# rpng/open_vins

Hardware: NVIDIA H100
Metric: msckf_updates_per_sec (higher is better)
Workload: dtype f64

## Files before the change

open_vins_b200/csrc/k_triangulate.cu:

```cuda
#include "geom.cuh"

__global__ void k_cam_poses(const DevFrame *fr, DevCamPoses *cc) {
  OVB_PDL_ENTER();
  int idx = blockIdx.x * blockDim.x + threadIdx.x;
  int total = fr->n_cams * fr->n_clones;
  if (idx >= total)
    return;
  int cam = idx / fr->n_clones, cl = idx % fr->n_clones;
  dm3 R_ItoC = ld_m3(fr->cam_R[cam]);
  dv3 p_IinC = ld_v3(fr->cam_p[cam]);
  dm3 R_GtoI = ld_m3(fr->clone_R[cl]);
  dv3 p_IinG = ld_v3(fr->clone_p[cl]);
  dm3 R = mul33(R_ItoC, R_GtoI);
  dv3 p = sub3(p_IinG, mTv3(R, p_IinC));
#pragma unroll
  for (int i = 0; i < 9; i++)
    cc->cc_R[cam][cl][i] = R.m[i];
  cc->cc_p[cam][cl][0] = p.x;
  cc->cc_p[cam][cl][1] = p.y;
  cc->cc_p[cam][cl][2] = p.z;
}

void launch_cam_poses(ovb_ctx *ctx) {
  int total = OVB_MAX_CAMS * OVB_MAX_CLONES;
  k_cam_poses<<<(total + 127) / 128, 128, 0, ctx->stream>>>(ctx->d_frame, ctx->d_cc);
}

#define TRI_MAX_WARPS 8
#define TRI_PITCH 33
template <int NV> __device__ __forceinline__ void seq_add(double (&s)[NV], const double (&c)[NV], int count, double *wbuf) {
  const int lane = threadIdx.x & 31;
#pragma unroll
  for (int k = 0; k < NV; k++)
    wbuf[k * TRI_PITCH + lane] = c[k];
  __syncwarp();
  double a = 0.0;
#pragma unroll
  for (int k = 0; k < NV; k++)
    a = (lane == k) ? s[k] : a;
  if (lane < NV) {
    const double *row = wbuf + lane * TRI_PITCH;
    for (int l = 0; l < count; l++)
      a += row[l];
  }
#pragma unroll
  for (int k = 0; k < NV; k++)
    s[k] = __shfl_sync(0xffffffffu, a, k);
  __syncwarp();
}

struct Rel {
  dm3 R;
  dv3 t;
  dv3 q;
};
__device__ __forceinline__ Rel rel_pose(const DevCamPoses *fr, int cam, int cl, const dm3 &R_GtoA, dv3 p_AinG) {
  dm3 Rc = ld_m3(fr->cc_R[cam][cl]);
  dv3 pc = ld_v3(fr->cc_p[cam][cl]);
  Rel r;
  r.R = mul33T(Rc, R_GtoA);
  r.t = mv3(R_GtoA, sub3(pc, p_AinG));
  r.q = negmv3(r.R, r.t);
  return r;
}

__device__ __forceinline__ double lm_cost(const DevCamPoses *fr, const BlobView &bv, int m0, int m1, int lane, const dm3 &R_GtoA, dv3 p_AinG,
                                          double alpha, double beta, double rho, double *wbuf) {
  double err[1] = {0.0};
  for (int base = m0; base < m1; base += 32) {
    const int i = base + lane;
    double c[1] = {0.0};
    if (i < m1) {
      Rel r = rel_pose(fr, bv.cam[i], bv.clone[i], R_GtoA, p_AinG);
      double hi1 = r.R.m[0] * alpha + r.R.m[1] * beta + r.R.m[2] + rho * r.q.x;
      double hi2 = r.R.m[3] * alpha + r.R.m[4] * beta + r.R.m[5] + rho * r.q.y;
      double hi3 = r.R.m[6] * alpha + r.R.m[7] * beta + r.R.m[8] + rho * r.q.z;
      float z0 = (float)(hi1 / hi3), z1 = (float)(hi2 / hi3);
      float r0 = __fsub_rn(bv.uvn[2 * i], z0), r1 = __fsub_rn(bv.uvn[2 * i + 1], z1);
      float nrm = __fsqrt_rn(__fadd_rn(__fmul_rn(r0, r0), __fmul_rn(r1, r1)));
      c[0] = (double)nrm * (double)nrm;
    }
    seq_add<1>(err, c, min(32, m1 - base), wbuf);
  }
  return err[0];
}

__global__ void __launch_bounds__(256) k_triangulate(const DevCamPoses *__restrict__ fr, const DevOpts *__restrict__ dop,
                                                     DevFeat *__restrict__ feats, int n_feats, BlobView bv) {
  OVB_PDL_ENTER();
  __shared__ double tri_stage[TRI_MAX_WARPS][9 * TRI_PITCH];
  double *wbuf = tri_stage[threadIdx.x >> 5];
  int warp = (blockIdx.x * blockDim.x + threadIdx.x) >> 5;
  int lane = threadIdx.x & 31;
  if (warp >= n_feats)
    return;
  DevFeat *F = &feats[warp];
  const ovb_opts &op = dop->o;
  int m0 = F->m0, m1 = F->m1;
  const double qnan = __longlong_as_double(0x7ff8000000000000LL);
  int status = OVB_FEAT_OK;
  dv3 pA = mk3(qnan, qnan, qnan), pG = pA;
  int anchor_cam = -1, anchor_clone = -1;
  if (m1 - m0 < 2) {
    status = OVB_FEAT_FEW_MEAS;
  } else {
    int most = 0;
    anchor_cam = 0;
    for (int k = F->key0; k < F->key1; k++) {
      int key = bv.keys[k];
      int cnt = 0;
      for (int i = m0 + lane; i < m1; i += 32)
        cnt += (bv.cam[i] == key) ? 1 : 0;
#pragma unroll
      for (int o = 16; o > 0; o >>= 1)
        cnt += __shfl_xor_sync(0xffffffffu, cnt, o);
      if (cnt > most) {
        anchor_cam = key;
        most = cnt;
      }
    }
    int ameas = -1;
    for (int i = m0 + lane; i < m1; i += 32)
      if (bv.cam[i] == anchor_cam)
        ameas = i;
#pragma unroll
    for (int o = 16; o > 0; o >>= 1)
      ameas = max(ameas, __shfl_xor_sync(0xffffffffu, ameas, o));
    anchor_clone = bv.clone[ameas];
    dm3 R_GtoA = ld_m3(fr->cc_R[anchor_cam][anchor_clone]);
    dv3 p_AinG = ld_v3(fr->cc_p[anchor_cam][anchor_clone]);
    dv3 p_f;
    if (!op.triangulate_1d) {
      double Ab[9] = {0, 0, 0, 0, 0, 0, 0, 0, 0};
      for (int base = m0; base < m1; base += 32) {
        const int i = base + lane;
        double c[9] = {0, 0, 0, 0, 0, 0, 0, 0, 0};
        if (i < m1) {
          Rel r = rel_pose(fr, bv.cam[i], bv.clone[i], R_GtoA, p_AinG);
          dv3 bi = mTv3(r.R, mk3((double)bv.uvn[2 * i], (double)bv.uvn[2 * i + 1], 1.0));
          double nb = norm3(bi);
          bi = mk3(bi.x / nb, bi.y / nb, bi.z / nb);
          dm3 Bp = skew3(bi);
          dm3 Ai = mulT33(Bp, Bp);
          dv3 Aip = mv3(Ai, r.t);
          c[0] = Ai.m[0], c[1] = Ai.m[1], c[2] = Ai.m[2], c[3] = Ai.m[4], c[4] = Ai.m[5], c[5] = Ai.m[8];
          c[6] = Aip.x, c[7] = Aip.y, c[8] = Aip.z;
        }
        seq_add<9>(Ab, c, min(32, m1 - base), wbuf);
      }
      double A[9] = {Ab[0], Ab[1], Ab[2], Ab[1], Ab[3], Ab[4], Ab[2], Ab[4], Ab[5]};
      double b[3] = {Ab[6], Ab[7], Ab[8]};
      p_f = colpiv_solve3(A, mk3(b[0], b[1], b[2]));
      double condA = cond_sym3(A);
      if (fabs(condA) > op.max_cond_number)
        status = OVB_FEAT_TRI_COND;
      else if (p_f.z < op.min_dist || p_f.z > op.max_dist)
        status = OVB_FEAT_TRI_DEPTH;
      else if (isnan(norm3(p_f)))
        status = OVB_FEAT_TRI_NAN;
    } else {
      dv3 ba = mk3((double)bv.uvn[2 * ameas], (double)bv.uvn[2 * ameas + 1], 1.0);
      double nba = norm3(ba);
      ba = mk3(ba.x / nba, ba.y / nba, ba.z / nba);
      double Ab1[2] = {0.0, 0.0};
      for (int base = m0; base < m1; base += 32) {
        const int i = base + lane;
        double c[2] = {0.0, 0.0};
        if (i < m1 && i != ameas) {
          Rel r = rel_pose(fr, bv.cam[i], bv.clone[i], R_GtoA, p_AinG);
          dv3 bi = mTv3(r.R, mk3((double)bv.uvn[2 * i], (double)bv.uvn[2 * i + 1], 1.0));
          double nb = norm3(bi);
          bi = mk3(bi.x / nb, bi.y / nb, bi.z / nb);
          dm3 Bp = skew3(bi);
          dv3 Bb = mv3(Bp, ba);
          c[0] = dot3(Bb, Bb);
          c[1] = dot3(Bb, mv3(Bp, r.t));
        }
        seq_add<2>(Ab1, c, min(32, m1 - base), wbuf);
      }
      const double A1 = Ab1[0], b1 = Ab1[1];
      double depth = b1 / A1;
      p_f = mk3(depth * ba.x, depth * ba.y, depth * ba.z);
      if (p_f.z < op.min_dist || p_f.z > op.max_dist)
        status = OVB_FEAT_TRI_DEPTH;
      else if (isnan(norm3(p_f)))
        status = OVB_FEAT_TRI_NAN;
    }
    if (status == OVB_FEAT_OK) {
      pA = p_f;
      pG = add3(mTv3(R_GtoA, pA), p_AinG);
    }
    if (status == OVB_FEAT_OK && op.refine_features) {
      double rho = 1 / pA.z;
      double alpha = pA.x / pA.z;
      double beta = pA.y / pA.z;
      double lam = op.init_lamda;
      double eps = 10000;
      int runs = 0;
      bool recompute = true;
      double Hs[6] = {0, 0, 0, 0, 0, 0};
      double g[3] = {0, 0, 0};
      double cost_old = lm_cost(fr, bv, m0, m1, lane, R_GtoA, p_AinG, alpha, beta, rho, wbuf);
      while (runs < op.max_runs && lam < op.max_lamda && eps > op.min_dx) {
        if (recompute) {
#pragma unroll
          for (int k = 0; k < 6; k++)
            Hs[k] = 0.0;
          g[0] = g[1] = g[2] = 0.0;
          double Hg[9] = {0, 0, 0, 0, 0, 0, 0, 0, 0};
          for (int base = m0; base < m1; base += 32) {
            const int i = base + lane;
            double c[9] = {0, 0, 0, 0, 0, 0, 0, 0, 0};
            if (i < m1) {
              Rel r = rel_pose(fr, bv.cam[i], bv.clone[i], R_GtoA, p_AinG);
              double hi1 = r.R.m[0] * alpha + r.R.m[1] * beta + r.R.m[2] + rho * r.q.x;
              double hi2 = r.R.m[3] * alpha + r.R.m[4] * beta + r.R.m[5] + rho * r.q.y;
              double hi3 = r.R.m[6] * alpha + r.R.m[7] * beta + r.R.m[8] + rho * r.q.z;
              double h3sq = hi3 * hi3;
              double H0[3], H1[3];
              H0[0] = (r.R.m[0] * hi3 - hi1 * r.R.m[6]) / h3sq;
              H0[1] = (r.R.m[1] * hi3 - hi1 * r.R.m[7]) / h3sq;
              H0[2] = (r.q.x * hi3 - hi1 * r.q.z) / h3sq;
              H1[0] = (r.R.m[3] * hi3 - hi2 * r.R.m[6]) / h3sq;
              H1[1] = (r.R.m[4] * hi3 - hi2 * r.R.m[7]) / h3sq;
              H1[2] = (r.q.y * hi3 - hi2 * r.q.z) / h3sq;
              float z0 = (float)(hi1 / hi3), z1 = (float)(hi2 / hi3);
              double rd0 = (double)__fsub_rn(bv.uvn[2 * i], z0), rd1 = (double)__fsub_rn(bv.uvn[2 * i + 1], z1);
              c[0] = H0[0] * H0[0] + H1[0] * H1[0];
              c[1] = H0[0] * H0[1] + H1[0] * H1[1];
              c[2] = H0[0] * H0[2] + H1[0] * H1[2];
              c[3] = H0[1] * H0[1] + H1[1] * H1[1];
              c[4] = H0[1] * H0[2] + H1[1] * H1[2];
              c[5] = H0[2] * H0[2] + H1[2] * H1[2];
#pragma unroll
              for (int a = 0; a < 3; a++)
                c[6 + a] = H0[a] * rd0 + H1[a] * rd1;
            }
            seq_add<9>(Hg, c, min(32, m1 - base), wbuf);
          }
#pragma unroll
          for (int k = 0; k < 6; k++)
            Hs[k] = Hg[k];
#pragma unroll
          for (int k = 0; k < 3; k++)
            g[k] = Hg[6 + k];
        }
        double Hl[9] = {Hs[0] * (1.0 + lam), Hs[1], Hs[2], Hs[1], Hs[3] * (1.0 + lam), Hs[4], Hs[2], Hs[4], Hs[5] * (1.0 + lam)};
        dv3 dx = colpiv_solve3(Hl, mk3(g[0], g[1], g[2]));
        double cost = lm_cost(fr, bv, m0, m1, lane, R_GtoA, p_AinG, alpha + dx.x, beta + dx.y, rho + dx.z, wbuf);
        if (cost <= cost_old && (cost_old - cost) / cost_old < op.min_dcost) {
          alpha += dx.x;
          beta += dx.y;
          rho += dx.z;
          eps = 0;
          break;
        }
        if (cost <= cost_old) {
          recompute = true;
          cost_old = cost;
          alpha += dx.x;
          beta += dx.y;
          rho += dx.z;
          runs++;
          lam = lam / op.lam_mult;
          eps = norm3(dx);
        } else {
          recompute = false;
          lam = lam * op.lam_mult;
        }
      }
      pA = mk3(alpha / rho, beta / rho, 1 / rho);
      dv3 q1, q2;
      householder_tangent3(pA, q1, q2);
      double base_line_max = 0.0;
      for (int i = m0 + lane; i < m1; i += 32) {
        dv3 pc = ld_v3(fr->cc_p[bv.cam[i]][bv.clone[i]]);
        dv3 t = mv3(R_GtoA, sub3(pc, p_AinG));
        double a0 = dot3(q1, t), a1 = dot3(q2, t);
        double bl = sqrt(a0 * a0 + a1 * a1);
        if (bl > base_line_max)
          base_line_max = bl;
      }
      base_line_max = warp_max(base_line_max);
      if (pA.z < op.min_dist || pA.z > op.max_dist)
        status = OVB_FEAT_GN_DEPTH;
      else if ((norm3(pA) / base_line_max) > op.max_baseline)
        status = OVB_FEAT_GN_BASELINE;
      else if (isnan(norm3(pA)))
        status = OVB_FEAT_GN_NAN;
      else
        pG = add3(mTv3(R_GtoA, pA), p_AinG);
    }
  }
  if (lane == 0) {
    F->status = status;
    F->anchor_cam = anchor_cam;
    F->anchor_clone = anchor_clone;
    F->p_FinA[0] = pA.x;
    F->p_FinA[1] = pA.y;
    F->p_FinA[2] = pA.z;
    F->p_FinG[0] = pG.x;
    F->p_FinG[1] = pG.y;
    F->p_FinG[2] = pG.z;
    F->chi2 = qnan;
  }
}

void launch_triangulate(ovb_ctx *ctx, int n_feats, BlobView bv) {
  if (n_feats <= 0)
    return;
  int warps_per_cta = (n_feats + ctx->sm_count - 1) / ctx->sm_count;
  warps_per_cta = warps_per_cta < 1 ? 1 : (warps_per_cta > 8 ? 8 : warps_per_cta);
  int grid = (n_feats + warps_per_cta - 1) / warps_per_cta;
  ovb_launch(ctx, k_triangulate, dim3(grid), dim3(warps_per_cta * 32), (size_t)(0), ctx->d_cc, ctx->d_opts, ctx->d_feat, n_feats, bv);
}
```

open_vins_b200/csrc/ovb_api.cu:

```cuda
#include "ovb_internal.cuh"
#include <chrono>
#include <algorithm>
#include <cmath>
#include <cstdio>
#include <cstdlib>
#include <cstring>
#include <new>
#include <vector>

static const double g_chi2_table[OVB_CHI2_TABLE_LEN] = {
#include "chi2_table.inc"
};

unsigned char *ovb_feat_order_ptr(ovb_ctx *ctx) { return ctx->d_feat_order; }

static size_t align_up(size_t v, size_t a) { return (v + a - 1) / a * a; }

extern "C" {

static ovb_status ensure_stage(ovb_ctx *ctx, size_t doubles);

int ovb_abi_version(void) { return OVB_ABI_VERSION; }

double ovb_chi2_quantile95(int dof) {
// ... 96 lines not shown
  ctx->off_opts = align_up(sizeof(DevFrame), 256);
  ctx->off_feat = ctx->off_opts + align_up(sizeof(DevOpts), 256);
  ctx->off_blob = ctx->off_feat + align_up(sizeof(DevFeat) * (size_t)ctx->cfg.max_feats, 256);
  ctx->blob_cap = align_up((size_t)ctx->cfg.max_meas * (1 + 2 + 8 + 8) + (size_t)ctx->cfg.max_feats * OVB_MAX_CAMS + 64, 256);
  ctx->arena_bytes = ctx->off_blob + ctx->blob_cap;
  CK(cudaMalloc(&ctx->d_arena, ctx->arena_bytes));
  CK(cudaMallocHost(&ctx->h_arena, ctx->arena_bytes));
  ctx->d_frame = (DevFrame *)ctx->d_arena;
  ctx->d_opts = (DevOpts *)(ctx->d_arena + ctx->off_opts);
  ctx->d_feat = (DevFeat *)(ctx->d_arena + ctx->off_feat);
  ctx->d_blob = ctx->d_arena + ctx->off_blob;
  ctx->h_frame = (DevFrame *)ctx->h_arena;
  ctx->h_opts = (DevOpts *)(ctx->h_arena + ctx->off_opts);
  ctx->h_feat = (DevFeat *)(ctx->h_arena + ctx->off_feat);
  ctx->h_blob = ctx->h_arena + ctx->off_blob;
  CK(cudaMalloc(&ctx->d_cc, sizeof(DevCamPoses)));
  CK(cudaMalloc(&ctx->d_feat_order, (size_t)ctx->cfg.max_feats * (OVB_MAX_VARS + 1)));
  ctx->info_bytes = align_up(sizeof(DevUpdateInfo), 256);
  CK(cudaMalloc(&ctx->d_info, ctx->info_bytes + sizeof(double) * (size_t)ms));
  ctx->d_dx = (double *)((char *)ctx->d_info + ctx->info_bytes);
  CK(cudaMallocHost(&ctx->h_info, ctx->info_bytes + sizeof(double) * (size_t)ms));
  ctx->h_dx = (double *)((char *)ctx->h_info + ctx->info_bytes);
  CK(cudaMalloc(&ctx->d_chi2_table, sizeof(g_chi2_table)));
  CK(cudaMemcpy(ctx->d_chi2_table, g_chi2_table, sizeof(g_chi2_table), cudaMemcpyHostToDevice));
  ctx->max_rows = ctx->cfg.max_rows > 0 ? ctx->cfg.max_rows : 2 * ctx->cfg.max_meas;
  if (ctx->max_rows < 2 * ctx->cfg.max_meas)
    ctx->max_rows = 2 * ctx->cfg.max_meas;
  int ldcap = std::min(OVB_MAX_COLS, ms) + 8;
  ctx->Hs_cap = (size_t)ctx->max_rows * ldcap;
  CK(cudaMalloc(&ctx->d_Hs, sizeof(double) * ctx->Hs_cap));
  ctx->h_stage = nullptr;
// ... 21 lines not shown
#undef CK
  *out = ctx;
  return OVB_OK;
}

void ovb_destroy(ovb_ctx *ctx) {
  if (ctx)
    for (int i = 0; i < 2 * 96; i++)
      if (ctx->prof_ev[i])
        cudaEventDestroy(ctx->prof_ev[i]);
  if (!ctx)
    return;
  cudaSetDevice(ctx->device);
  if (ctx->stream)
    cudaStreamSynchronize(ctx->stream);
  void *dev[] = {ctx->P[0],   ctx->P[1], ctx->d_arena, ctx->d_cc, ctx->d_feat_order, ctx->d_info, ctx->d_chi2_table, ctx->d_Hs, ctx->d_W[0],
                 ctx->d_W[1], ctx->d_R,  ctx->d_R2,    ctx->d_M,  ctx->d_S,          ctx->d_Y,    ctx->d_w,          ctx->d_scratch,
                 ctx->d_long, ctx->d_dump, ctx->P_snap, ctx->d_flush, ctx->d_Gpart, ctx->d_G, ctx->d_cqw, ctx->d_grp, ctx->d_grp_acc, ctx->d_init, ctx->d_imu, ctx->d_pub};
  for (void *p : dev)
    if (p)
      cudaFree(p);
  void *host[] = {ctx->h_arena, ctx->h_info, ctx->h_stage, ctx->h_grp, ctx->h_init, ctx->h_imu};
  for (void *p : host)
    if (p)
      cudaFreeHost(p);
  for (int i = 0; i < 8; i++)
    if (ctx->ev[i])
      cudaEventDestroy(ctx->ev[i]);
  if (ctx->ev_fork)
    cudaEventDestroy(ctx->ev_fork);
  if (ctx->ev_join)
// ... 826 lines not shown
  stats->ms_total = ctx->stage_ms[5];
}

ovb_status ovb_triangulate(ovb_ctx *ctx, const ovb_frame *frame, const ovb_feat_batch *feats, const ovb_opts *opts, ovb_feat_out *out) {
  if (!ctx || !out)
    return OVB_ERR_ARG;
  OVB_CUDA_CHECK(ctx, cudaSetDevice(ctx->device));
  Packed pk;
  int saveN = ctx->N;
  if (ctx->N == 0)
    ctx->N = ctx->cfg.max_state;
  ovb_status st = pack_inputs(ctx, frame, feats, opts, nullptr, &pk, nullptr, false);
  ctx->N = saveN;
  if (st != OVB_OK)
    return st;
  launch_cam_poses(ctx);
  launch_triangulate(ctx, pk.n_feats, pk.bv);
  OVB_CUDA_CHECK(ctx, cudaGetLastError());
  OVB_CUDA_CHECK(ctx, cudaMemcpyAsync(ctx->h_feat, ctx->d_feat, sizeof(DevFeat) * (size_t)pk.n_feats, cudaMemcpyDeviceToHost, ctx->stream));
  OVB_CUDA_CHECK(ctx, cudaStreamSynchronize(ctx->stream));
  unpack_feats(ctx, pk.n_feats, out);
  return OVB_OK;
}

ovb_status ovb_feature_jacobians(ovb_ctx *ctx, const ovb_frame *frame, const ovb_feat_batch *feats, const ovb_opts *opts, ovb_feat_out *out,
                                 int stage, double *Hf_out, double *Hx_out, double *res_out, int32_t *row_off_out, int32_t *ncols_out,
                                 int32_t *col_index_out, int ld_out) {
  if (!ctx || !out || !row_off_out || !ncols_out || !col_index_out)
    return OVB_ERR_ARG;
  if (ctx->N < 1) {
    snprintf(ctx->err, sizeof(ctx->err), "ovb_feature_jacobians: no covariance loaded (ovb_cov_set)");
    return OVB_ERR_ARG;
  }
  OVB_CUDA_CHECK(ctx, cudaSetDevice(ctx->device));
  Packed pk;
  ovb_status st = pack_inputs(ctx, frame, feats, opts, out, &pk);
  if (st != OVB_OK)
    return st;
  const int F = pk.n_feats, n_all = pk.n_all;
  if (ld_out < n_all)
    return OVB_ERR_ARG;
  *ncols_out = n_all;
  for (int s = 0, c = 0; s < ctx->h_frame->n_slots; s++)
    for (int k = 0; k < ctx->h_frame->slot_size[s]; k++)
      col_index_out[c++] = ctx->h_frame->slot_off[s] + k;
  launch_cam_poses(ctx);
  if (stage == 0) {
    int rows = 2 * pk.n_meas;
    size_t need = (size_t)rows * (OVB_MAX_COLS + 4);
    if (!ctx->d_dump || need > ctx->dump_cap) {
      if (ctx->d_dump)
        cudaFree(ctx->d_dump);
      ctx->dump_cap = need;
      OVB_CUDA_CHECK(ctx, cudaMalloc(&ctx->d_dump, sizeof(double) * ctx->dump_cap));
    }
    ctx->dump_rows = rows;
    OVB_CUDA_CHECK(ctx, cudaMemsetAsync(ctx->d_dump, 0, sizeof(double) * need, ctx->stream));
    launch_feature_system(ctx, F, pk.bv, pk.ldH, 1);
    OVB_CUDA_CHECK(ctx, cudaGetLastError());
    std::vector<double> host(need);
    OVB_CUDA_CHECK(ctx, cudaMemcpyAsync(host.data(), ctx->d_dump, sizeof(double) * need, cudaMemcpyDeviceToHost, ctx->stream));
// ... 92 lines not shown
  int64_t *cnt = ctx->init_counters;
  cnt[0] = cnt[1] = cnt[2] = cnt[3] = 0;
  OVB_CUDA_CHECK(ctx, cudaSetDevice(ctx->device));
  Packed pk;
  const int saveN = ctx->N;
  if (ctx->N == 0)
    ctx->N = ctx->cfg.max_state;
  ovb_status st = pack_inputs(ctx, frame, feats, opts, nullptr, &pk, nullptr, false, feat_rep, sigma_pix, chi2_multipler);
  ctx->N = saveN;
  if (st != OVB_OK)
    return st;
  st = feature_scratch_reserve(ctx, F, false, true);
  if (st != OVB_OK)
    return st;
  cnt[2] += (int64_t)ctx->last_h2d_bytes;
  launch_cam_poses(ctx);
  launch_triangulate(ctx, F, pk.bv);
  OVB_CUDA_CHECK(ctx, cudaGetLastError());
  OVB_CUDA_CHECK(ctx, cudaMemcpyAsync(ctx->h_feat, ctx->d_feat, sizeof(DevFeat) * (size_t)F, cudaMemcpyDeviceToHost, ctx->stream));
  OVB_CUDA_CHECK(ctx, cudaStreamSynchronize(ctx->stream));
  cnt[1]++;
  cnt[3] += (int64_t)(sizeof(DevFeat) * (size_t)F);
  unpack_feats(ctx, F, out);
  if (!ctx->d_init) {
    OVB_CUDA_CHECK(ctx, cudaMalloc(&ctx->d_init, sizeof(DevInitSys)));
    OVB_CUDA_CHECK(ctx, cudaMallocHost(&ctx->h_init, sizeof(DevInitSys)));
  }
  std::vector<int> sched_of(F);
  for (int i = 0; i < F; i++)
    sched_of[ctx->h_feat[i].sched] = i;
  const DevFrame *hf = ctx->h_frame;
// ... 31 lines not shown
      seen |= 1ull << hf->clone_slot[d.anchor_clone];
      if (opts->do_calib_camera_pose && hf->cam_ext_slot[d.anchor_cam] >= 0)
        seen |= 1ull << hf->cam_ext_slot[d.anchor_cam];
    }
    int n = 0;
    for (int s = 0; s < hf->n_slots; s++)
      if ((seen >> s) & 1ull)
        n += hf->slot_size[s];
    if (n > ctx->cfg.max_state)
      return OVB_ERR_CAPACITY;
    cnt[0]++;
    if (moved) {
      copy_frame_values(ctx->h_frame, frame);
      OVB_CUDA_CHECK(ctx, cudaMemcpyAsync(ctx->d_frame, ctx->h_frame, sizeof(DevFrame), cudaMemcpyHostToDevice, ctx->stream));
      cnt[2] += (int64_t)sizeof(DevFrame);
      launch_cam_poses(ctx);
    }
    launch_feature_init(ctx, sched_of[f], pk.bv, pk.ldH);
    launch_init_prep(ctx, f, k, n);
    const int *skip = &ctx->d_init->skip;
    if (!launch_cov_init_augment(ctx, k, n, ctx->d_init->HR, ctx->d_init->Hinv, d.sigma_sq, skip)) {
      snprintf(ctx->err, sizeof(ctx->err), "ovb_slam_delayed_init: covariance augmentation kernel could not be launched (N=%d, k=%d)", N0, k);
      return OVB_ERR_CAPACITY;
    }
    const double *Hdev = ctx->d_Hs + (size_t)d.row0 * pk.ldH;
    const int rows = 2 * (d.m1 - d.m0) - 3;
    int rr = rows;
    if (rows > n) {
      rr = compress_system(ctx, OVB_COMPRESS_CHOLQR2, ctx->d_Hs + (size_t)d.row0 * pk.ldH, rows, n, pk.ldH, ctx->d_R, pk.ldH);
      Hdev = ctx->d_R;
    }
// ... 97 lines not shown
    return n;
  if (mode == OVB_COMPRESS_NORMAL_EQUATIONS && launch_compress_gram(ctx, A, m, n, ldA, Rout, ldR) >= 0)
    return n;
  launch_tsqr(ctx, A, m, n, ldA, Rout, ldR);
  return std::min(m, n);
}

static int enqueue_slam_groups(ovb_ctx *ctx, int n_groups, int ldH);
static int enqueue_update(ovb_ctx *ctx, const Packed &pk, int col_order, cudaEvent_t *ev, bool slam = false) {
  const int N = ctx->N, F = pk.n_feats, ldH = pk.ldH, m_total = pk.m_total, n_all = pk.n_all, n_groups = pk.n_groups;
  const BlobView bv = pk.bv;
  ctx->n_launch = 0;
  ctx->n_launch_tsqr_level = 0;
  ctx->prof_n = 0;
  if (!slam) {
    launch_cam_poses(ctx);
    launch_triangulate(ctx, F, bv);
    ctx->n_launch += 2;
  }
  ctx->n_launch += 1;
  if (ev)
    cudaEventRecord(ev[1], ctx->stream);
  launch_feature_system(ctx, F, bv, ldH, slam ? 2 : 0);
  if (ev)
    cudaEventRecord(ev[2], ctx->stream);
  {
    cudaEventRecord(ctx->ev_fork, ctx->stream);
    cudaStreamWaitEvent(ctx->side_stream, ctx->ev_fork, 0);
    cudaStream_t main_stream = ctx->stream;
    ctx->stream = ctx->side_stream;
    if (slam) {
      launch_column_map_slam(ctx, F, n_groups == 1);
    } else {
// ... 380 lines not shown
  cudaEventRecord(ctx->ev[0], ctx->stream);
  Packed pk;
  ovb_opts o2 = *opts;
  o2.col_order = OVB_COLS_CANONICAL;
  ovb_status st = pack_inputs(ctx, frame, feats, &o2, nullptr, &pk);
  if (st != OVB_OK)
    return st;
  cudaEventRecord(ctx->ev[1], ctx->stream);
  *n_cols = pk.n_all;
  *ld = pk.ldH;
  if ((size_t)pk.n_all * pk.ldH > (size_t)R_cap_doubles)
    return OVB_ERR_CAPACITY;
  ctx->last_pk = pk;
  ctx->n_launch = 0;
  ctx->n_launch_tsqr_level = 0;
  launch_cam_poses(ctx);
  launch_triangulate(ctx, pk.n_feats, pk.bv);
  launch_feature_system(ctx, pk.n_feats, pk.bv, pk.ldH, 0);
  launch_column_map(ctx, pk.n_feats, pk.bv);
  ctx->n_launch += 3;
  if (pk.m_total > 0)
    compress_system(ctx, o2.compress, ctx->d_Hs, pk.m_total, pk.n_all, pk.ldH, R_dev, pk.ldH);
  else
    OVB_CUDA_CHECK(ctx, cudaMemsetAsync(R_dev, 0, sizeof(double) * (size_t)pk.n_all * pk.ldH, ctx->stream));
  cudaEventRecord(ctx->ev[4], ctx->stream);
  OVB_CUDA_CHECK(ctx, cudaGetLastError());
  return OVB_OK;
}

ovb_status ovb_msckf_shard_finish(ovb_ctx *ctx, double *stacked_dev, int n_blocks, ovb_feat_out *out, double *dx, ovb_stats *stats) {
  if (!ctx || !stacked_dev || n_blocks < 1 || !dx || ctx->N < 1)
// ... 344 lines not shown
```

open_vins_b200/csrc/ovb_internal.cuh:

```cuda
#pragma once
#include "../../include/ovb200.h"
#include <cuda_runtime.h>
#include <stdint.h>

#define OVB_BIG_MAX_MEAS 128
#define OVB_MAX_COLS 512
#define OVB_NB 16
#define OVB_CR 256
#define OVB_PROP_MAX_N 64
#define OVB_PROP_STEPS_RESERVE 64
#define OVB_NO_NEG_DIAG 0x7fffffff

struct DevFrame {
  int n_clones, n_cams;
  int n_slots;
  int n_all;
  double clone_R[OVB_MAX_CLONES][9];
  double clone_p[OVB_MAX_CLONES][3];
  double clone_R_fej[OVB_MAX_CLONES][9];
  double clone_p_fej[OVB_MAX_CLONES][3];
  double cam_R[OVB_MAX_CAMS][9];
  double cam_p[OVB_MAX_CAMS][3];
  double cam_intr[OVB_MAX_CAMS][8];
  int cam_model[OVB_MAX_CAMS];
// ... 3 lines not shown
  int clone_slot[OVB_MAX_CLONES];
  int cam_ext_slot[OVB_MAX_CAMS];
  int cam_intr_slot[OVB_MAX_CAMS];
  const struct DevGroup *groups;
  int lm_w;
};

struct DevGroup {
  int f0, f1;
  int row0, rows;
  int n_cols;
  int n_ent;
  int ent[OVB_MAX_VARS + OVB_MAX_COLS];
  int col_state[OVB_MAX_COLS];
  short col_frame[OVB_MAX_COLS];
};

struct DevCamPoses {
  double cc_R[OVB_MAX_CAMS][OVB_MAX_CLONES][9];
  double cc_p[OVB_MAX_CAMS][OVB_MAX_CLONES][3];
};

struct DevOpts {
  ovb_opts o;
  double sigma_pix_sq;
  int rep;
};

struct DevFeat {
  int m0, m1;
  int row0;
  int key0, key1;
  int status;
  int anchor_cam, anchor_clone;
  int sched;
// ... 83 lines not shown
  char err[256];
  int N, ldP;
  double *P[2];
  int cur;
  unsigned char *d_arena, *h_arena;
  size_t arena_bytes, off_opts, off_feat, off_blob;
  DevFrame *d_frame;
  DevOpts *d_opts;
  DevFeat *d_feat;
  unsigned char *d_blob;
  DevFrame *h_frame;
  DevOpts *h_opts;
  DevFeat *h_feat;
  unsigned char *h_blob;
  size_t blob_cap;
  DevCamPoses *d_cc;
  unsigned char *d_feat_order;
  DevUpdateInfo *d_info;
  DevUpdateInfo *h_info;
  double *h_dx;
  double *h_stage;
  size_t stage_cap;
  double *d_chi2_table;
  double *d_Hs;
  size_t Hs_cap;
  double *d_W[2];
  size_t W_cap;
  double *d_R;
  double *d_R2;
  double *d_M;
  double *d_S;
  double *d_Y;
  double *d_w;
  double *d_dx;
  double *d_scratch;
  size_t scratch_per_cta;
  int scratch_ctas;
  double *d_long;
  size_t long_cap;
  double *d_dump;
  size_t dump_cap;
  int dump_rows;
  int max_rows;
  int sm_count;
  size_t info_bytes;
  int attr_done[8];
  int tsqr_pdl;
  int tsqr_cluster;
  int gram_cluster;
  int ekf_chol_dmma;
  mutable float stage_ms[6];
  mutable int stage_pending;
  double host_us[4];
  int replay_enabled, last_pk_valid;
  Packed last_pk;
  int last_col_order;
  double *P_snap;
  void *d_flush;
  DevGroup *d_grp, *h_grp;
  int grp_cap;
  double *d_grp_acc;
// ... 12 lines not shown
  size_t imu_cap;
  int prof_on, prof_n;
  cudaEvent_t prof_ev[2 * 96];
  const void *prof_fn[96];
};

#define OVB_CUDA_CHECK(ctx, call)                                                                                     \
  do {                                                                                                                \
    cudaError_t e_ = (call);                                                                                          \
    if (e_ != cudaSuccess) {                                                                                          \
      snprintf((ctx)->err, sizeof((ctx)->err), "%s:%d %s: %s", __FILE__, __LINE__, #call, cudaGetErrorString(e_));    \
      return OVB_ERR_CUDA;                                                                                            \
    }                                                                                                                 \
  } while (0)

void launch_cam_poses(ovb_ctx *ctx);
void launch_triangulate(ovb_ctx *ctx, int n_feats, BlobView bv);
void launch_feature_system(ovb_ctx *ctx, int n_feats, BlobView bv, int ldH, int mode);
ovb_status feature_scratch_reserve(ovb_ctx *ctx, int n_feats, bool slam, bool init = false);
void launch_feature_init(ovb_ctx *ctx, int sched, BlobView bv, int ldH);
void launch_init_prep(ovb_ctx *ctx, int feat, int k, int n);
void launch_column_map(ovb_ctx *ctx, int n_feats, BlobView bv, int rows_drop = 3);
void launch_column_map_slam(ovb_ctx *ctx, int n_feats, bool full_map);
void launch_tsqr(ovb_ctx *ctx, double *A, int m, int n, int ldA, double *Rout, int ldR);
int launch_compress_gram(ovb_ctx *ctx, const double *A, int m, int n, int ldA, double *Rout, int ldR);
int launch_compress_cholqr2(ovb_ctx *ctx, double *A, int m, int n, int ldA, double *Rout, int ldR);
bool launch_chol_ekf_dmma(ovb_ctx *ctx, double *S, int ldS, int r, const double *res, double *w, double *invdiag, double **Lpk_out,
                          unsigned long long *epoch_out);
bool launch_trsm_rows(ovb_ctx *ctx, double *A, int ldA, int m, int nt, const double *Lpk, unsigned long long epoch);
bool launch_chol_solve_wide(ovb_ctx *ctx, double *S, int ldS, int r, double *w, double *invdiag, double *M, int ldM, int N, bool gate_only);
void launch_reorder_R(ovb_ctx *ctx, const double *Rin, int n_all, int ldRin, double *Rout, int ldRout);
// ... 44 lines not shown
```

Measured before the change: 2576.

## Fuse camera-pose kernel into triangulation and cache relative poses in shared memory

Removes the separate k_cam_poses launch and computes camera poses inline inside the triangulation kernel. Each warp now computes per-measurement relative poses once into dynamic shared memory, and reuses them across the linear solve, every Levenberg-Marquardt pass and the baseline check, instead of recomputing them each time. The LM step also merges the cost and Hessian passes so the initial cost comes from the Hessian pass. The price is that the host must scan the features for the largest measurement count to size shared memory, and large features can limit warps per CTA. An optional compile-time probe adds clock64 phase timing.

```diff
diff --git a/open_vins_b200/csrc/k_triangulate.cu b/open_vins_b200/csrc/k_triangulate.cu
--- a/open_vins_b200/csrc/k_triangulate.cu
+++ b/open_vins_b200/csrc/k_triangulate.cu
@@ -1,46 +1,96 @@
 #include "geom.cuh"
-
-__global__ void k_cam_poses(const DevFrame *fr, DevCamPoses *cc) {
-  OVB_PDL_ENTER();
-  int idx = blockIdx.x * blockDim.x + threadIdx.x;
-  int total = fr->n_cams * fr->n_clones;
-  if (idx >= total)
+#ifdef TRI_PROBE
+#include <cstdio>
+#endif
+
+#ifdef TRI_PROBE
+#define TRI_PROBE_FEATS 8192
+#define TRI_PROBE_EV 40
+struct TriProbe {
+  long long t0, t1;
+  long long beg[TRI_PROBE_EV], end[TRI_PROBE_EV];
+  char lbl[TRI_PROBE_EV];
+  int n, M, acc, rej;
+};
+__device__ TriProbe tri_probe[TRI_PROBE_FEATS];
+__device__ unsigned tri_probe_done;
+#define TRI_P_DECL long long tp_b = clock64(); int tp_n = 0, tp_acc = 0, tp_rej = 0; \
+  TriProbe *tp = (warp < TRI_PROBE_FEATS && lane == 0) ? &tri_probe[warp] : nullptr; if (tp) tp->t0 = tp_b
+#define TRI_P_BEGIN() do { tp_b = clock64(); } while (0)
+#define TRI_P_END(c) do { long long e_ = clock64(); if (tp && tp_n < TRI_PROBE_EV) { tp->beg[tp_n] = tp_b; tp->end[tp_n] = e_; tp->lbl[tp_n] = (c); } tp_n++; } while (0)
+#define TRI_P_ACC() (tp_acc++)
+#define TRI_P_REJ() (tp_rej++)
+#define TRI_P_FINISH() tri_probe_finish(tp, warp, lane, n_feats, tp_n, m1 - m0, tp_acc, tp_rej)
+__device__ __noinline__ void tri_probe_finish(TriProbe *tp, int warp, int lane, int n_feats, int n, int M, int acc, int rej) {
+  if (lane != 0)
     return;
-  int cam = idx / fr->n_clones, cl = idx % fr->n_clones;
+  if (tp) {
+    tp->t1 = clock64();
+    tp->n = n < TRI_PROBE_EV ? n : TRI_PROBE_EV;
+    tp->M = M, tp->acc = acc, tp->rej = rej;
+  }
+  __threadfence();
+  if (atomicAdd(&tri_probe_done, 1u) != (unsigned)n_feats - 1)
+    return;
+  __threadfence();
+  const int nf = n_feats < TRI_PROBE_FEATS ? n_feats : TRI_PROBE_FEATS;
+  int w = 0;
+  long long sum = 0;
+  for (int f = 0; f < nf; f++) {
+    const long long t = tri_probe[f].t1 - tri_probe[f].t0;
+    sum += t;
+    if (t > tri_probe[w].t1 - tri_probe[w].t0)
+      w = f;
+  }
+  const TriProbe &p = tri_probe[w];
+  long long ph[8] = {0, 0, 0, 0, 0, 0, 0, 0};
+  int npass = 0;
+  for (int k = 0; k < p.n; k++) {
+    const long long d = p.end[k] - p.beg[k];
+    const char c = p.lbl[k];
+    ph[c == 'a' ? 0 : c == 'l' ? 1 : c == 'c' ? 2 : (c == 'S' || c == 'H') ? 3 : c == 'A' ? 4 : c == 'R' ? 5 : 6] += d;
+    npass += (c == 'S' || c == 'H' || c == 'A' || c == 'R') ? 1 : 0;
+  }
+  long long tracked = 0;
+  for (int k = 0; k < 7; k++)
+    tracked += ph[k];
+  printf("TRI_PROBE n_feats=%d mean_warp=%lld longest warp=%d M=%d a=%d r=%d passes=%d total=%lld | anchor %lld linear %lld cond %lld "
+         "start+Hessian %lld trial-acc %lld trial-rej %lld baseline %lld other %lld\n",
+         n_feats, sum / nf, w, p.M, p.acc, p.rej, npass, p.t1 - p.t0, ph[0], ph[1], ph[2], ph[3], ph[4], ph[5], ph[6], p.t1 - p.t0 - tracked);
+  for (int k = 0; k < p.n; k++)
+    printf("TRI_PROBE   %c %lld\n", p.lbl[k], p.end[k] - p.beg[k]);
+  tri_probe_done = 0;
+}
+#else
+#define TRI_P_DECL do { } while (0)
+#define TRI_P_BEGIN() do { } while (0)
+#define TRI_P_END(c) do { } while (0)
+#define TRI_P_ACC() do { } while (0)
+#define TRI_P_REJ() do { } while (0)
+#define TRI_P_FINISH() do { } while (0)
+#endif
+
+__device__ __forceinline__ void cam_pose(const DevFrame *fr, int cam, int cl, dm3 &R, dv3 &p) {
   dm3 R_ItoC = ld_m3(fr->cam_R[cam]);
   dv3 p_IinC = ld_v3(fr->cam_p[cam]);
   dm3 R_GtoI = ld_m3(fr->clone_R[cl]);
   dv3 p_IinG = ld_v3(fr->clone_p[cl]);
-  dm3 R = mul33(R_ItoC, R_GtoI);
-  dv3 p = sub3(p_IinG, mTv3(R, p_IinC));
-#pragma unroll
-  for (int i = 0; i < 9; i++)
-    cc->cc_R[cam][cl][i] = R.m[i];
-  cc->cc_p[cam][cl][0] = p.x;
-  cc->cc_p[cam][cl][1] = p.y;
-  cc->cc_p[cam][cl][2] = p.z;
-}
-
-void launch_cam_poses(ovb_ctx *ctx) {
-  int total = OVB_MAX_CAMS * OVB_MAX_CLONES;
-  k_cam_poses<<<(total + 127) / 128, 128, 0, ctx->stream>>>(ctx->d_frame, ctx->d_cc);
-}
-
-#define TRI_MAX_WARPS 8
-#define TRI_PITCH 33
-template <int NV> __device__ __forceinline__ void seq_add(double (&s)[NV], const double (&c)[NV], int count, double *wbuf) {
+  R = mul33(R_ItoC, R_GtoI);
+  p = sub3(p_IinG, mTv3(R, p_IinC));
+}
+
+#define TRI_REL 15
+#define TRI_NC 10
+#define TRI_APOSE 12
+#define TRI_SMEM_LIMIT (227 * 1024)
+
+template <int NV> __device__ __forceinline__ void seq_sum(double (&s)[NV], const double *stg, int pitch, int M) {
   const int lane = threadIdx.x & 31;
-#pragma unroll
-  for (int k = 0; k < NV; k++)
-    wbuf[k * TRI_PITCH + lane] = c[k];
   __syncwarp();
   double a = 0.0;
-#pragma unroll
-  for (int k = 0; k < NV; k++)
-    a = (lane == k) ? s[k] : a;
   if (lane < NV) {
-    const double *row = wbuf + lane * TRI_PITCH;
-    for (int l = 0; l < count; l++)
+    const double *row = stg + lane * pitch;
+    for (int l = 0; l < M; l++)
       a += row[l];
   }
 #pragma unroll
@@ -54,54 +104,89 @@
   dv3 t;
   dv3 q;
 };
-__device__ __forceinline__ Rel rel_pose(const DevCamPoses *fr, int cam, int cl, const dm3 &R_GtoA, dv3 p_AinG) {
-  dm3 Rc = ld_m3(fr->cc_R[cam][cl]);
-  dv3 pc = ld_v3(fr->cc_p[cam][cl]);
+__device__ __forceinline__ void rel_pose_store(const DevFrame *fr, int cam, int cl, const dm3 &R_GtoA, dv3 p_AinG, double *rel, int pitch) {
+  dm3 Rc;
+  dv3 pc;
+  cam_pose(fr, cam, cl, Rc, pc);
   Rel r;
   r.R = mul33T(Rc, R_GtoA);
   r.t = mv3(R_GtoA, sub3(pc, p_AinG));
   r.q = negmv3(r.R, r.t);
-  return r;
-}
-
-__device__ __forceinline__ double lm_cost(const DevCamPoses *fr, const BlobView &bv, int m0, int m1, int lane, const dm3 &R_GtoA, dv3 p_AinG,
-                                          double alpha, double beta, double rho, double *wbuf) {
-  double err[1] = {0.0};
-  for (int base = m0; base < m1; base += 32) {
-    const int i = base + lane;
-    double c[1] = {0.0};
-    if (i < m1) {
-      Rel r = rel_pose(fr, bv.cam[i], bv.clone[i], R_GtoA, p_AinG);
-      double hi1 = r.R.m[0] * alpha + r.R.m[1] * beta + r.R.m[2] + rho * r.q.x;
-      double hi2 = r.R.m[3] * alpha + r.R.m[4] * beta + r.R.m[5] + rho * r.q.y;
-      double hi3 = r.R.m[6] * alpha + r.R.m[7] * beta + r.R.m[8] + rho * r.q.z;
-      float z0 = (float)(hi1 / hi3), z1 = (float)(hi2 / hi3);
-      float r0 = __fsub_rn(bv.uvn[2 * i], z0), r1 = __fsub_rn(bv.uvn[2 * i + 1], z1);
-      float nrm = __fsqrt_rn(__fadd_rn(__fmul_rn(r0, r0), __fmul_rn(r1, r1)));
-      c[0] = (double)nrm * (double)nrm;
-    }
-    seq_add<1>(err, c, min(32, m1 - base), wbuf);
-  }
-  return err[0];
-}
-
-__global__ void __launch_bounds__(256) k_triangulate(const DevCamPoses *__restrict__ fr, const DevOpts *__restrict__ dop,
-                                                     DevFeat *__restrict__ feats, int n_feats, BlobView bv) {
+#pragma unroll
+  for (int k = 0; k < 9; k++)
+    rel[k * pitch] = r.R.m[k];
+  rel[9 * pitch] = r.t.x, rel[10 * pitch] = r.t.y, rel[11 * pitch] = r.t.z;
+  rel[12 * pitch] = r.q.x, rel[13 * pitch] = r.q.y, rel[14 * pitch] = r.q.z;
+}
+__device__ __forceinline__ dm3 rel_R(const double *rel, int pitch) {
+  dm3 R;
+#pragma unroll
+  for (int k = 0; k < 9; k++)
+    R.m[k] = rel[k * pitch];
+  return R;
+}
+__device__ __forceinline__ dv3 rel_t(const double *rel, int pitch) { return mk3(rel[9 * pitch], rel[10 * pitch], rel[11 * pitch]); }
+__device__ __forceinline__ dv3 rel_q(const double *rel, int pitch) { return mk3(rel[12 * pitch], rel[13 * pitch], rel[14 * pitch]); }
+
+template <bool HESS>
+__device__ __forceinline__ void lm_pass(double (&s)[HESS ? TRI_NC : 1], const BlobView &bv, int m0, int M, int lane, const double *rel, double *stg,
+                                        int pitch, double alpha, double beta, double rho) {
+  for (int j = lane; j < M; j += 32) {
+    const int i = m0 + j;
+    const dm3 R = rel_R(rel + j, pitch);
+    const dv3 q = rel_q(rel + j, pitch);
+    double hi1 = R.m[0] * alpha + R.m[1] * beta + R.m[2] + rho * q.x;
+    double hi2 = R.m[3] * alpha + R.m[4] * beta + R.m[5] + rho * q.y;
+    double hi3 = R.m[6] * alpha + R.m[7] * beta + R.m[8] + rho * q.z;
+    float z0 = (float)(hi1 / hi3), z1 = (float)(hi2 / hi3);
+    float r0 = __fsub_rn(bv.uvn[2 * i], z0), r1 = __fsub_rn(bv.uvn[2 * i + 1], z1);
+    float nrm = __fsqrt_rn(__fadd_rn(__fmul_rn(r0, r0), __fmul_rn(r1, r1)));
+    stg[j] = (double)nrm * (double)nrm;
+    if (HESS) {
+      double h3sq = hi3 * hi3;
+      double H0[3], H1[3];
+      H0[0] = (R.m[0] * hi3 - hi1 * R.m[6]) / h3sq;
+      H0[1] = (R.m[1] * hi3 - hi1 * R.m[7]) / h3sq;
+      H0[2] = (q.x * hi3 - hi1 * q.z) / h3sq;
+      H1[0] = (R.m[3] * hi3 - hi2 * R.m[6]) / h3sq;
+      H1[1] = (R.m[4] * hi3 - hi2 * R.m[7]) / h3sq;
+      H1[2] = (q.y * hi3 - hi2 * q.z) / h3sq;
+      double rd0 = (double)r0, rd1 = (double)r1;
+      stg[1 * pitch + j] = H0[0] * H0[0] + H1[0] * H1[0];
+      stg[2 * pitch + j] = H0[0] * H0[1] + H1[0] * H1[1];
+      stg[3 * pitch + j] = H0[0] * H0[2] + H1[0] * H1[2];
+      stg[4 * pitch + j] = H0[1] * H0[1] + H1[1] * H1[1];
+      stg[5 * pitch + j] = H0[1] * H0[2] + H1[1] * H1[2];
+      stg[6 * pitch + j] = H0[2] * H0[2] + H1[2] * H1[2];
+#pragma unroll
+      for (int a = 0; a < 3; a++)
+        stg[(7 + a) * pitch + j] = H0[a] * rd0 + H1[a] * rd1;
+    }
+  }
+  seq_sum<HESS ? TRI_NC : 1>(s, stg, pitch, M);
+}
+
+__global__ void __launch_bounds__(256) k_triangulate(const DevFrame *__restrict__ fr, const DevOpts *__restrict__ dop,
+                                                     DevFeat *__restrict__ feats, int n_feats, BlobView bv, int pitch) {
   OVB_PDL_ENTER();
-  __shared__ double tri_stage[TRI_MAX_WARPS][9 * TRI_PITCH];
-  double *wbuf = tri_stage[threadIdx.x >> 5];
+  extern __shared__ double tri_smem[];
+  double *rel = tri_smem + (size_t)(threadIdx.x >> 5) * ((TRI_REL + TRI_NC) * pitch + TRI_APOSE);
+  double *stg = rel + TRI_REL * pitch;
+  double *apose = stg + TRI_NC * pitch;
   int warp = (blockIdx.x * blockDim.x + threadIdx.x) >> 5;
   int lane = threadIdx.x & 31;
   if (warp >= n_feats)
     return;
+  TRI_P_DECL;
   DevFeat *F = &feats[warp];
   const ovb_opts &op = dop->o;
   int m0 = F->m0, m1 = F->m1;
+  const int M = m1 - m0;
   const double qnan = __longlong_as_double(0x7ff8000000000000LL);
   int status = OVB_FEAT_OK;
   dv3 pA = mk3(qnan, qnan, qnan), pG = pA;
   int anchor_cam = -1, anchor_clone = -1;
-  if (m1 - m0 < 2) {
+  if (M < 2) {
     status = OVB_FEAT_FEW_MEAS;
   } else {
     int most = 0;
@@ -127,31 +212,43 @@
     for (int o = 16; o > 0; o >>= 1)
       ameas = max(ameas, __shfl_xor_sync(0xffffffffu, ameas, o));
     anchor_clone = bv.clone[ameas];
-    dm3 R_GtoA = ld_m3(fr->cc_R[anchor_cam][anchor_clone]);
-    dv3 p_AinG = ld_v3(fr->cc_p[anchor_cam][anchor_clone]);
+    dm3 R_GtoA;
+    dv3 p_AinG;
+    cam_pose(fr, anchor_cam, anchor_clone, R_GtoA, p_AinG);
+    if (lane == 0) {
+#pragma unroll
+      for (int k = 0; k < 9; k++)
+        apose[k] = R_GtoA.m[k];
+      apose[9] = p_AinG.x, apose[10] = p_AinG.y, apose[11] = p_AinG.z;
+    }
+    for (int j = lane; j < M; j += 32)
+      rel_pose_store(fr, bv.cam[m0 + j], bv.clone[m0 + j], R_GtoA, p_AinG, rel + j, pitch);
+    TRI_P_END('a');
+    TRI_P_BEGIN();
     dv3 p_f;
     if (!op.triangulate_1d) {
-      double Ab[9] = {0, 0, 0, 0, 0, 0, 0, 0, 0};
-      for (int base = m0; base < m1; base += 32) {
-        const int i = base + lane;
-        double c[9] = {0, 0, 0, 0, 0, 0, 0, 0, 0};
-        if (i < m1) {
-          Rel r = rel_pose(fr, bv.cam[i], bv.clone[i], R_GtoA, p_AinG);
-          dv3 bi = mTv3(r.R, mk3((double)bv.uvn[2 * i], (double)bv.uvn[2 * i + 1], 1.0));
-          double nb = norm3(bi);
-          bi = mk3(bi.x / nb, bi.y / nb, bi.z / nb);
-          dm3 Bp = skew3(bi);
-          dm3 Ai = mulT33(Bp, Bp);
-          dv3 Aip = mv3(Ai, r.t);
-          c[0] = Ai.m[0], c[1] = Ai.m[1], c[2] = Ai.m[2], c[3] = Ai.m[4], c[4] = Ai.m[5], c[5] = Ai.m[8];
-          c[6] = Aip.x, c[7] = Aip.y, c[8] = Aip.z;
-        }
-        seq_add<9>(Ab, c, min(32, m1 - base), wbuf);
+      double Ab[9];
+      for (int j = lane; j < M; j += 32) {
+        const int i = m0 + j;
+        dv3 bi = mTv3(rel_R(rel + j, pitch), mk3((double)bv.uvn[2 * i], (double)bv.uvn[2 * i + 1], 1.0));
+        double nb = norm3(bi);
+        bi = mk3(bi.x / nb, bi.y / nb, bi.z / nb);
+        dm3 Bp = skew3(bi);
+        dm3 Ai = mulT33(Bp, Bp);
+        dv3 Aip = mv3(Ai, rel_t(rel + j, pitch));
+        const double c[9] = {Ai.m[0], Ai.m[1], Ai.m[2], Ai.m[4], Ai.m[5], Ai.m[8], Aip.x, Aip.y, Aip.z};
+#pragma unroll
+        for (int k = 0; k < 9; k++)
+          stg[k * pitch + j] = c[k];
       }
+      seq_sum<9>(Ab, stg, pitch, M);
       double A[9] = {Ab[0], Ab[1], Ab[2], Ab[1], Ab[3], Ab[4], Ab[2], Ab[4], Ab[5]};
       double b[3] = {Ab[6], Ab[7], Ab[8]};
       p_f = colpiv_solve3(A, mk3(b[0], b[1], b[2]));
+      TRI_P_END('l');
+      TRI_P_BEGIN();
       double condA = cond_sym3(A);
+      TRI_P_END('c');
       if (fabs(condA) > op.max_cond_number)
         status = OVB_FEAT_TRI_COND;
       else if (p_f.z < op.min_dist || p_f.z > op.max_dist)
@@ -162,25 +259,27 @@
       dv3 ba = mk3((double)bv.uvn[2 * ameas], (double)bv.uvn[2 * ameas + 1], 1.0);
       double nba = norm3(ba);
       ba = mk3(ba.x / nba, ba.y / nba, ba.z / nba);
-      double Ab1[2] = {0.0, 0.0};
-      for (int base = m0; base < m1; base += 32) {
-        const int i = base + lane;
+      double Ab1[2];
+      for (int j = lane; j < M; j += 32) {
+        const int i = m0 + j;
         double c[2] = {0.0, 0.0};
-        if (i < m1 && i != ameas) {
-          Rel r = rel_pose(fr, bv.cam[i], bv.clone[i], R_GtoA, p_AinG);
-          dv3 bi = mTv3(r.R, mk3((double)bv.uvn[2 * i], (double)bv.uvn[2 * i + 1], 1.0));
+        if (i != ameas) {
+          dv3 bi = mTv3(rel_R(rel + j, pitch), mk3((double)bv.uvn[2 * i], (double)bv.uvn[2 * i + 1], 1.0));
           double nb = norm3(bi);
           bi = mk3(bi.x / nb, bi.y / nb, bi.z / nb);
           dm3 Bp = skew3(bi);
           dv3 Bb = mv3(Bp, ba);
           c[0] = dot3(Bb, Bb);
-          c[1] = dot3(Bb, mv3(Bp, r.t));
+          c[1] = dot3(Bb, mv3(Bp, rel_t(rel + j, pitch)));
         }
-        seq_add<2>(Ab1, c, min(32, m1 - base), wbuf);
+        stg[j] = c[0];
+        stg[pitch + j] = c[1];
       }
+      seq_sum<2>(Ab1, stg, pitch, M);
       const double A1 = Ab1[0], b1 = Ab1[1];
       double depth = b1 / A1;
       p_f = mk3(depth * ba.x, depth * ba.y, depth * ba.z);
+      TRI_P_END('l');
       if (p_f.z < op.min_dist || p_f.z > op.max_dist)
         status = OVB_FEAT_TRI_DEPTH;
       else if (isnan(norm3(p_f)))
@@ -197,58 +296,28 @@
       double lam = op.init_lamda;
       double eps = 10000;
       int runs = 0;
-      bool recompute = true;
-      double Hs[6] = {0, 0, 0, 0, 0, 0};
-      double g[3] = {0, 0, 0};
-      double cost_old = lm_cost(fr, bv, m0, m1, lane, R_GtoA, p_AinG, alpha, beta, rho, wbuf);
+      double s[TRI_NC];
+      TRI_P_BEGIN();
+      lm_pass<true>(s, bv, m0, M, lane, rel, stg, pitch, alpha, beta, rho);
+      TRI_P_END('S');
+      double cost_old = s[0];
+      bool recompute = false;
       while (runs < op.max_runs && lam < op.max_lamda && eps > op.min_dx) {
         if (recompute) {
-#pragma unroll
-          for (int k = 0; k < 6; k++)
-            Hs[k] = 0.0;
-          g[0] = g[1] = g[2] = 0.0;
-          double Hg[9] = {0, 0, 0, 0, 0, 0, 0, 0, 0};
-          for (int base = m0; base < m1; base += 32) {
-            const int i = base + lane;
-            double c[9] = {0, 0, 0, 0, 0, 0, 0, 0, 0};
-            if (i < m1) {
-              Rel r = rel_pose(fr, bv.cam[i], bv.clone[i], R_GtoA, p_AinG);
-              double hi1 = r.R.m[0] * alpha + r.R.m[1] * beta + r.R.m[2] + rho * r.q.x;
-              double hi2 = r.R.m[3] * alpha + r.R.m[4] * beta + r.R.m[5] + rho * r.q.y;
-              double hi3 = r.R.m[6] * alpha + r.R.m[7] * beta + r.R.m[8] + rho * r.q.z;
-              double h3sq = hi3 * hi3;
-              double H0[3], H1[3];
-              H0[0] = (r.R.m[0] * hi3 - hi1 * r.R.m[6]) / h3sq;
-              H0[1] = (r.R.m[1] * hi3 - hi1 * r.R.m[7]) / h3sq;
-              H0[2] = (r.q.x * hi3 - hi1 * r.q.z) / h3sq;
-              H1[0] = (r.R.m[3] * hi3 - hi2 * r.R.m[6]) / h3sq;
-              H1[1] = (r.R.m[4] * hi3 - hi2 * r.R.m[7]) / h3sq;
-              H1[2] = (r.q.y * hi3 - hi2 * r.q.z) / h3sq;
-              float z0 = (float)(hi1 / hi3), z1 = (float)(hi2 / hi3);
-              double rd0 = (double)__fsub_rn(bv.uvn[2 * i], z0), rd1 = (double)__fsub_rn(bv.uvn[2 * i + 1], z1);
-              c[0] = H0[0] * H0[0] + H1[0] * H1[0];
-              c[1] = H0[0] * H0[1] + H1[0] * H1[1];
-              c[2] = H0[0] * H0[2] + H1[0] * H1[2];
-              c[3] = H0[1] * H0[1] + H1[1] * H1[1];
-              c[4] = H0[1] * H0[2] + H1[1] * H1[2];
-              c[5] = H0[2] * H0[2] + H1[2] * H1[2];
-#pragma unroll
-              for (int a = 0; a < 3; a++)
-                c[6 + a] = H0[a] * rd0 + H1[a] * rd1;
-            }
-            seq_add<9>(Hg, c, min(32, m1 - base), wbuf);
-          }
-#pragma unroll
-          for (int k = 0; k < 6; k++)
-            Hs[k] = Hg[k];
-#pragma unroll
-          for (int k = 0; k < 3; k++)
-            g[k] = Hg[6 + k];
+          TRI_P_BEGIN();
+          lm_pass<true>(s, bv, m0, M, lane, rel, stg, pitch, alpha, beta, rho);
+          TRI_P_END('H');
         }
+        const double Hs[6] = {s[1], s[2], s[3], s[4], s[5], s[6]};
         double Hl[9] = {Hs[0] * (1.0 + lam), Hs[1], Hs[2], Hs[1], Hs[3] * (1.0 + lam), Hs[4], Hs[2], Hs[4], Hs[5] * (1.0 + lam)};
-        dv3 dx = colpiv_solve3(Hl, mk3(g[0], g[1], g[2]));
-        double cost = lm_cost(fr, bv, m0, m1, lane, R_GtoA, p_AinG, alpha + dx.x, beta + dx.y, rho + dx.z, wbuf);
+        dv3 dx = colpiv_solve3(Hl, mk3(s[7], s[8], s[9]));
+        double cost_t[1];
+        TRI_P_BEGIN();
+        lm_pass<false>(cost_t, bv, m0, M, lane, rel, stg, pitch, alpha + dx.x, beta + dx.y, rho + dx.z);
+        const double cost = cost_t[0];
+        TRI_P_END(cost <= cost_old ? 'A' : 'R');
         if (cost <= cost_old && (cost_old - cost) / cost_old < op.min_dcost) {
+          TRI_P_ACC();
           alpha += dx.x;
           beta += dx.y;
           rho += dx.z;
@@ -264,24 +333,27 @@
           runs++;
           lam = lam / op.lam_mult;
           eps = norm3(dx);
+          TRI_P_ACC();
         } else {
+          TRI_P_REJ();
           recompute = false;
           lam = lam * op.lam_mult;
         }
       }
       pA = mk3(alpha / rho, beta / rho, 1 / rho);
+      TRI_P_BEGIN();
       dv3 q1, q2;
       householder_tangent3(pA, q1, q2);
       double base_line_max = 0.0;
-      for (int i = m0 + lane; i < m1; i += 32) {
-        dv3 pc = ld_v3(fr->cc_p[bv.cam[i]][bv.clone[i]]);
-        dv3 t = mv3(R_GtoA, sub3(pc, p_AinG));
+      for (int j = lane; j < M; j += 32) {
+        dv3 t = rel_t(rel + j, pitch);
         double a0 = dot3(q1, t), a1 = dot3(q2, t);
         double bl = sqrt(a0 * a0 + a1 * a1);
         if (bl > base_line_max)
           base_line_max = bl;
       }
       base_line_max = warp_max(base_line_max);
+      TRI_P_END('b');
       if (pA.z < op.min_dist || pA.z > op.max_dist)
         status = OVB_FEAT_GN_DEPTH;
       else if ((norm3(pA) / base_line_max) > op.max_baseline)
@@ -289,7 +361,7 @@
       else if (isnan(norm3(pA)))
         status = OVB_FEAT_GN_NAN;
       else
-        pG = add3(mTv3(R_GtoA, pA), p_AinG);
+        pG = add3(mTv3(ld_m3(apose), pA), ld_v3(apose + 9));
     }
   }
   if (lane == 0) {
@@ -304,13 +376,28 @@
     F->p_FinG[2] = pG.z;
     F->chi2 = qnan;
   }
+  TRI_P_FINISH();
 }
 
 void launch_triangulate(ovb_ctx *ctx, int n_feats, BlobView bv) {
   if (n_feats <= 0)
     return;
+  if (!ctx->attr_done[8]) {
+    cudaFuncSetAttribute(k_triangulate, cudaFuncAttributeMaxDynamicSharedMemorySize, TRI_SMEM_LIMIT);
+    ctx->attr_done[8] = 1;
+  }
+  int maxM = 2;
+  for (int f = 0; f < n_feats; f++) {
+    const int M = ctx->h_feat[f].m1 - ctx->h_feat[f].m0;
+    maxM = M > maxM ? M : maxM;
+  }
+  const int pitch = maxM | 1;
+  const size_t per_warp = sizeof(double) * ((TRI_REL + TRI_NC) * (size_t)pitch + TRI_APOSE);
+  const int fit = (int)(TRI_SMEM_LIMIT / per_warp);
   int warps_per_cta = (n_feats + ctx->sm_count - 1) / ctx->sm_count;
   warps_per_cta = warps_per_cta < 1 ? 1 : (warps_per_cta > 8 ? 8 : warps_per_cta);
+  warps_per_cta = warps_per_cta > fit ? fit : warps_per_cta;
   int grid = (n_feats + warps_per_cta - 1) / warps_per_cta;
-  ovb_launch(ctx, k_triangulate, dim3(grid), dim3(warps_per_cta * 32), (size_t)(0), ctx->d_cc, ctx->d_opts, ctx->d_feat, n_feats, bv);
-}
+  ovb_launch(ctx, k_triangulate, dim3(grid), dim3(warps_per_cta * 32), per_warp * warps_per_cta, ctx->d_frame, ctx->d_opts, ctx->d_feat, n_feats, bv,
+             pitch);
+}
diff --git a/open_vins_b200/csrc/ovb_api.cu b/open_vins_b200/csrc/ovb_api.cu
--- a/open_vins_b200/csrc/ovb_api.cu
+++ b/open_vins_b200/csrc/ovb_api.cu
@@ -134,7 +134,6 @@
   ctx->h_opts = (DevOpts *)(ctx->h_arena + ctx->off_opts);
   ctx->h_feat = (DevFeat *)(ctx->h_arena + ctx->off_feat);
   ctx->h_blob = ctx->h_arena + ctx->off_blob;
-  CK(cudaMalloc(&ctx->d_cc, sizeof(DevCamPoses)));
   CK(cudaMalloc(&ctx->d_feat_order, (size_t)ctx->cfg.max_feats * (OVB_MAX_VARS + 1)));
   ctx->info_bytes = align_up(sizeof(DevUpdateInfo), 256);
   CK(cudaMalloc(&ctx->d_info, ctx->info_bytes + sizeof(double) * (size_t)ms));
@@ -186,7 +185,7 @@
   cudaSetDevice(ctx->device);
   if (ctx->stream)
     cudaStreamSynchronize(ctx->stream);
-  void *dev[] = {ctx->P[0],   ctx->P[1], ctx->d_arena, ctx->d_cc, ctx->d_feat_order, ctx->d_info, ctx->d_chi2_table, ctx->d_Hs, ctx->d_W[0],
+  void *dev[] = {ctx->P[0],   ctx->P[1], ctx->d_arena, ctx->d_feat_order, ctx->d_info, ctx->d_chi2_table, ctx->d_Hs, ctx->d_W[0],
                  ctx->d_W[1], ctx->d_R,  ctx->d_R2,    ctx->d_M,  ctx->d_S,          ctx->d_Y,    ctx->d_w,          ctx->d_scratch,
                  ctx->d_long, ctx->d_dump, ctx->P_snap, ctx->d_flush, ctx->d_Gpart, ctx->d_G, ctx->d_cqw, ctx->d_grp, ctx->d_grp_acc, ctx->d_init, ctx->d_imu, ctx->d_pub};
   for (void *p : dev)
@@ -1043,7 +1042,6 @@
   ctx->N = saveN;
   if (st != OVB_OK)
     return st;
-  launch_cam_poses(ctx);
   launch_triangulate(ctx, pk.n_feats, pk.bv);
   OVB_CUDA_CHECK(ctx, cudaGetLastError());
   OVB_CUDA_CHECK(ctx, cudaMemcpyAsync(ctx->h_feat, ctx->d_feat, sizeof(DevFeat) * (size_t)pk.n_feats, cudaMemcpyDeviceToHost, ctx->stream));
@@ -1073,7 +1071,6 @@
   for (int s = 0, c = 0; s < ctx->h_frame->n_slots; s++)
     for (int k = 0; k < ctx->h_frame->slot_size[s]; k++)
       col_index_out[c++] = ctx->h_frame->slot_off[s] + k;
-  launch_cam_poses(ctx);
   if (stage == 0) {
     int rows = 2 * pk.n_meas;
     size_t need = (size_t)rows * (OVB_MAX_COLS + 4);
@@ -1196,7 +1193,6 @@
   if (st != OVB_OK)
     return st;
   cnt[2] += (int64_t)ctx->last_h2d_bytes;
-  launch_cam_poses(ctx);
   launch_triangulate(ctx, F, pk.bv);
   OVB_CUDA_CHECK(ctx, cudaGetLastError());
   OVB_CUDA_CHECK(ctx, cudaMemcpyAsync(ctx->h_feat, ctx->d_feat, sizeof(DevFeat) * (size_t)F, cudaMemcpyDeviceToHost, ctx->stream));
@@ -1258,7 +1254,6 @@
       copy_frame_values(ctx->h_frame, frame);
       OVB_CUDA_CHECK(ctx, cudaMemcpyAsync(ctx->d_frame, ctx->h_frame, sizeof(DevFrame), cudaMemcpyHostToDevice, ctx->stream));
       cnt[2] += (int64_t)sizeof(DevFrame);
-      launch_cam_poses(ctx);
     }
     launch_feature_init(ctx, sched_of[f], pk.bv, pk.ldH);
     launch_init_prep(ctx, f, k, n);
@@ -1386,9 +1381,8 @@
   ctx->n_launch_tsqr_level = 0;
   ctx->prof_n = 0;
   if (!slam) {
-    launch_cam_poses(ctx);
     launch_triangulate(ctx, F, bv);
-    ctx->n_launch += 2;
+    ctx->n_launch += 1;
   }
   ctx->n_launch += 1;
   if (ev)
@@ -1799,7 +1793,6 @@
   ctx->last_pk = pk;
   ctx->n_launch = 0;
   ctx->n_launch_tsqr_level = 0;
-  launch_cam_poses(ctx);
   launch_triangulate(ctx, pk.n_feats, pk.bv);
   launch_feature_system(ctx, pk.n_feats, pk.bv, pk.ldH, 0);
   launch_column_map(ctx, pk.n_feats, pk.bv);
diff --git a/open_vins_b200/csrc/ovb_internal.cuh b/open_vins_b200/csrc/ovb_internal.cuh
--- a/open_vins_b200/csrc/ovb_internal.cuh
+++ b/open_vins_b200/csrc/ovb_internal.cuh
@@ -41,11 +41,6 @@
   int ent[OVB_MAX_VARS + OVB_MAX_COLS];
   int col_state[OVB_MAX_COLS];
   short col_frame[OVB_MAX_COLS];
-};
-
-struct DevCamPoses {
-  double cc_R[OVB_MAX_CAMS][OVB_MAX_CLONES][9];
-  double cc_p[OVB_MAX_CAMS][OVB_MAX_CLONES][3];
 };
 
 struct DevOpts {
@@ -159,7 +154,6 @@
   DevFeat *h_feat;
   unsigned char *h_blob;
   size_t blob_cap;
-  DevCamPoses *d_cc;
   unsigned char *d_feat_order;
   DevUpdateInfo *d_info;
   DevUpdateInfo *h_info;
@@ -189,7 +183,7 @@
   int max_rows;
   int sm_count;
   size_t info_bytes;
-  int attr_done[8];
+  int attr_done[9];
   int tsqr_pdl;
   int tsqr_cluster;
   int gram_cluster;
@@ -232,7 +226,6 @@
     }                                                                                                                 \
   } while (0)
 
-void launch_cam_poses(ovb_ctx *ctx);
 void launch_triangulate(ovb_ctx *ctx, int n_feats, BlobView bv);
 void launch_feature_system(ovb_ctx *ctx, int n_feats, BlobView bv, int ldH, int mode);
 ovb_status feature_scratch_reserve(ovb_ctx *ctx, int n_feats, bool slam, bool init = false);
```

Measured after the change: 2622, median of 6. +1.8%, better.
